# benfred/implicit

Measured on NVIDIA H100. Metric: ALS user+item row-updates/sec at f=64, higher is better.
Workload: dtype f32 (tensor-core accumulation with 3-term hi/lo splits, fp32-faithful)

## Files before the change

implicit_b200/csrc/cholesky_device.cuh:

```cuda
#pragma once
#include <limits.h>
#include <stdlib.h>

#include <cuda_fp16.h>

#include "common.h"

namespace als {

namespace {

__device__ __forceinline__ void mma_tf32(float (&d)[4], uint32_t a0, uint32_t a1, uint32_t a2, uint32_t a3,
                                         uint32_t b0, uint32_t b1) {
  asm volatile(
      "mma.sync.aligned.m16n8k8.row.col.f32.tf32.tf32.f32 {%0,%1,%2,%3}, {%4,%5,%6,%7}, {%8,%9}, {%0,%1,%2,%3};\n"
      : "+f"(d[0]), "+f"(d[1]), "+f"(d[2]), "+f"(d[3])
      : "r"(a0), "r"(a1), "r"(a2), "r"(a3), "r"(b0), "r"(b1));
}

__device__ __forceinline__ void cp_async16(float *smem_dst, const float *gmem_src) {
  const uint32_t s = (uint32_t)__cvta_generic_to_shared(smem_dst);
  asm volatile("cp.async.cg.shared.global [%0], [%1], 16;\n" ::"r"(s), "l"(gmem_src) : "memory");
}
__device__ __forceinline__ void cp_async_commit() { asm volatile("cp.async.commit_group;\n" ::: "memory"); }
template <int N>
__device__ __forceinline__ void cp_async_wait() {
  asm volatile("cp.async.wait_group %0;\n" ::"n"(N) : "memory");
}

constexpr uint32_t kTf32Mask = 0xffffe000u;
constexpr uint32_t kSignBit = 0x80000000u;

__device__ __forceinline__ uint32_t rn_tf32(float x) { return (__float_as_uint(x) + 0x1000u) & kTf32Mask; }
__device__ __forceinline__ void split_tf32(float x, uint32_t &hi, uint32_t &lo) {
  hi = rn_tf32(x);
  lo = __float_as_uint(x - __uint_as_float(hi));
}

__device__ __forceinline__ float rcp_approx(float x) {
  float r;
  asm("rcp.approx.ftz.f32 %0, %1;" : "=f"(r) : "f"(x));
  return r;
}
__device__ __forceinline__ float rsqrt_approx(float x) {
  float r;
  asm("rsqrt.approx.ftz.f32 %0, %1;" : "=f"(r) : "f"(x));
  return r;
}

template <int NB>
struct Cfg {
  static constexpr int F = 16 * NB;
  static constexpr int NT8 = 2 * NB;
  static constexpr int NTILES = NB * (NB + 1);
  static constexpr int LDS = F + 8;
  static constexpr int NSTAGE = 3;
  static constexpr int STAGE_FLOATS = 8 * LDS + 16;
  __host__ __device__ static constexpr int pstride(int p) { return F - 8 * p + ((p & 1) ? 0 : 8); }
  __host__ __device__ static constexpr int poff(int p) {
    int o = 0;
    for (int q = 0; q < p; ++q) o += 8 * pstride(q);
    return o;
  }
  static constexpr int U_FLOATS = poff(NT8);
  static constexpr int WARP_FLOATS = NSTAGE * STAGE_FLOATS + U_FLOATS + F ;
  __host__ __device__ static constexpr int tidx(int i, int j) { return i * NT8 - i * (i - 1) + (j - 2 * i); }
  static constexpr int SLOT_FLOATS = 32 * (NTILES * 4 + NT8);
};

constexpr int kWarpsPerCta = 1;

template <int NB>
struct RowState {
  float acc[Cfg<NB>::NTILES][4];
  float bp[Cfg<NB>::NT8];
};

struct Blk {
  int idx;
  float c;
};

__device__ __forceinline__ Blk load_block(const WorkItem &wi, int b, const int32_t *__restrict__ indices,
                                          const float *__restrict__ data, int lane) {
  const int k = wi.k0 + 32 * b + lane;
  const bool valid = k < wi.k1;
  Blk r;
  r.idx = valid ? __ldg(indices + k) : -1;
  r.c = valid ? __ldg(data + k) : 0.f;
  return r;
}

template <int NB>
__device__ __forceinline__ void issue_kstep(float *stage, const Blk &blk, int s, bool active,
                                            const float *__restrict__ Y, int lane) {
  using C = Cfg<NB>;
  if (active) {
    const int src = 8 * s + (lane & 7);
    const float c = __shfl_sync(0xffffffffu, blk.c, src);
    const int myidx = __shfl_sync(0xffffffffu, blk.idx, src);
    if (lane < 8) {
      const float w = (myidx >= 0) ? fabsf(c) - 1.f : 0.f;
      stage[8 * C::LDS + lane] = copysignf(__fsqrt_rn(fabsf(w)), w);
      stage[8 * C::LDS + 8 + lane] = (myidx >= 0 && c > 0.f) ? c : 0.f;
    }
    const int first = __shfl_sync(0xffffffffu, blk.idx, 8 * s);
    constexpr int CH = C::F / 4;
#pragma unroll
    for (int q = 0; q < NB; ++q) {
      const int id = q * 32 + lane;
      const int row = id / CH, ch = id % CH;
      int ridx = __shfl_sync(0xffffffffu, blk.idx, 8 * s + row);
      if (ridx < 0) ridx = first;
      cp_async16(stage + row * C::LDS + ch * 4, Y + (int64_t)ridx * C::F + ch * 4);
    }
  }
  cp_async_commit();
}

template <int NB>
__device__ __forceinline__ void consume_kstep(RowState<NB> &st, const float *stage, int g, int t) {
  using C = Cfg<NB>;
  const float s0 = stage[8 * C::LDS + t], s1 = stage[8 * C::LDS + t + 4];
  const float c0 = stage[8 * C::LDS + 8 + t], c1 = stage[8 * C::LDS + 8 + t + 4];
  const float a0 = fabsf(s0), a1 = fabsf(s1);
  const uint32_t m0 = __float_as_uint(s0) & kSignBit, m1 = __float_as_uint(s1) & kSignBit;
  uint32_t vh0[C::NT8], vl0[C::NT8], vh1[C::NT8], vl1[C::NT8];
#pragma unroll
  for (int c = 0; c < C::NT8; ++c) {
    const float y0 = stage[t * C::LDS + 8 * c + g];
    const float y1 = stage[(t + 4) * C::LDS + 8 * c + g];
    st.bp[c] = fmaf(c0, y0, st.bp[c]);
    st.bp[c] = fmaf(c1, y1, st.bp[c]);
    split_tf32(a0 * y0, vh0[c], vl0[c]);
    split_tf32(a1 * y1, vh1[c], vl1[c]);
  }
#pragma unroll
  for (int term = 0; term < 3; ++term) {
#pragma unroll
    for (int i = 0; i < NB; ++i) {
      const uint32_t a0 = (term == 0 ? vl0[2 * i] : vh0[2 * i]) ^ m0;
      const uint32_t a1 = (term == 0 ? vl0[2 * i + 1] : vh0[2 * i + 1]) ^ m0;
      const uint32_t a2 = (term == 0 ? vl1[2 * i] : vh1[2 * i]) ^ m1;
      const uint32_t a3 = (term == 0 ? vl1[2 * i + 1] : vh1[2 * i + 1]) ^ m1;
#pragma unroll
      for (int j = 2 * i; j < C::NT8; ++j) {
        float(&d)[4] = st.acc[C::tidx(i, j)];
        if (term == 1) mma_tf32(d, a0, a1, a2, a3, vl0[j], vl1[j]);
        else mma_tf32(d, a0, a1, a2, a3, vh0[j], vh1[j]);
      }
    }
  }
}

__device__ __forceinline__ void mma_f16(float (&d)[4], uint32_t a0, uint32_t a1, uint32_t a2, uint32_t a3, uint32_t b0,
                                        uint32_t b1) {
  asm volatile(
      "mma.sync.aligned.m16n8k16.row.col.f32.f16.f16.f32 {%0,%1,%2,%3}, {%4,%5,%6,%7}, {%8,%9}, {%0,%1,%2,%3};\n"
      : "+f"(d[0]), "+f"(d[1]), "+f"(d[2]), "+f"(d[3])
      : "r"(a0), "r"(a1), "r"(a2), "r"(a3), "r"(b0), "r"(b1));
}

__device__ __forceinline__ void split_f16_pair(float x0, float x1, uint32_t &hi, uint32_t &lo) {
  const __half2 h = __floats2half2_rn(x0, x1);
  const float2 hf = __half22float2(h);
  const __half2 l = __floats2half2_rn(x0 - hf.x, x1 - hf.y);
  hi = *reinterpret_cast<const uint32_t *>(&h);
  lo = *reinterpret_cast<const uint32_t *>(&l);
}

__device__ __forceinline__ float pow2_scale_below_2_14(float p) {
  const unsigned b = __float_as_uint(p);
  const int E = (int)(b >> 23) & 0xff;
  int se = (b & 0x7fffffffu) ? 267 - E : 127;
  se = se < 1 ? 1 : se > 253 ? 253 : se;
  return __uint_as_float((unsigned)se << 23);
}

template <int NB>
struct Cfg16 {
  using C = Cfg<NB>;
  static constexpr int F = C::F;
  static constexpr int LDS = F + 4;
  static constexpr int NSTAGE = 2;
  static constexpr int STAGE_FLOATS = 16 * LDS + 32;
  static constexpr int WARP_FLOATS = NSTAGE * STAGE_FLOATS + C::U_FLOATS + F ;
};

template <int NB>
__device__ __forceinline__ void issue_kstep16(float *stage, const Blk &blk, int s2, bool active, float sigma,
                                              const float *__restrict__ Y, int lane) {
  using C = Cfg16<NB>;
  if (active) {
    const int src = 16 * s2 + (lane & 15);
    const float c = __shfl_sync(0xffffffffu, blk.c, src);
    const int myidx = __shfl_sync(0xffffffffu, blk.idx, src);
    if (lane < 16) {
      const float w = (myidx >= 0) ? fabsf(c) - 1.f : 0.f;
      stage[16 * C::LDS + lane] = copysignf(sigma * __fsqrt_rn(fabsf(w)), w);
      stage[16 * C::LDS + 16 + lane] = (myidx >= 0 && c > 0.f) ? c : 0.f;
    }
    const int first = __shfl_sync(0xffffffffu, blk.idx, 16 * s2);
    constexpr int CH = C::F / 4;
#pragma unroll
    for (int q = 0; q < 2 * NB; ++q) {
      const int id = q * 32 + lane;
      const int row = id / CH, ch = id % CH;
      int ridx = __shfl_sync(0xffffffffu, blk.idx, 16 * s2 + row);
      if (ridx < 0) ridx = first;
      cp_async16(stage + row * C::LDS + ch * 4, Y + (int64_t)ridx * C::F + ch * 4);
    }
  }
  cp_async_commit();
}

template <int NB>
__device__ __forceinline__ void consume_kstep16(RowState<NB> &st, const float *stage, int g, int t) {
  using C = Cfg<NB>;
  constexpr int LDS = Cfg16<NB>::LDS;
  const float2 s0 = *reinterpret_cast<const float2 *>(stage + 16 * LDS + 2 * t);
  const float2 s1 = *reinterpret_cast<const float2 *>(stage + 16 * LDS + 2 * t + 8);
  const float2 c0 = *reinterpret_cast<const float2 *>(stage + 16 * LDS + 16 + 2 * t);
  const float2 c1 = *reinterpret_cast<const float2 *>(stage + 16 * LDS + 16 + 2 * t + 8);
  const float a00 = fabsf(s0.x), a01 = fabsf(s0.y), a10 = fabsf(s1.x), a11 = fabsf(s1.y);
  const uint32_t m0 = ((__float_as_uint(s0.x) >> 16) & 0x8000u) | (__float_as_uint(s0.y) & kSignBit);
  const uint32_t m1 = ((__float_as_uint(s1.x) >> 16) & 0x8000u) | (__float_as_uint(s1.y) & kSignBit);
  uint32_t h0[C::NT8], l0[C::NT8], h1[C::NT8], l1[C::NT8];
  const float *r00 = stage + (2 * t) * LDS + g, *r01 = r00 + LDS, *r10 = r00 + 8 * LDS, *r11 = r10 + LDS;
#pragma unroll
  for (int c = 0; c < C::NT8; ++c) {
    const float y00 = r00[8 * c], y01 = r01[8 * c], y10 = r10[8 * c], y11 = r11[8 * c];
    st.bp[c] = fmaf(c0.x, y00, st.bp[c]);
    st.bp[c] = fmaf(c0.y, y01, st.bp[c]);
    st.bp[c] = fmaf(c1.x, y10, st.bp[c]);
    st.bp[c] = fmaf(c1.y, y11, st.bp[c]);
    split_f16_pair(a00 * y00, a01 * y01, h0[c], l0[c]);
    split_f16_pair(a10 * y10, a11 * y11, h1[c], l1[c]);
  }
#pragma unroll
  for (int term = 0; term < 3; ++term) {
#pragma unroll
    for (int i = 0; i < NB; ++i) {
      const uint32_t a0 = (term == 0 ? l0[2 * i] : h0[2 * i]) ^ m0;
      const uint32_t a1 = (term == 0 ? l0[2 * i + 1] : h0[2 * i + 1]) ^ m0;
      const uint32_t a2 = (term == 0 ? l1[2 * i] : h1[2 * i]) ^ m1;
      const uint32_t a3 = (term == 0 ? l1[2 * i + 1] : h1[2 * i + 1]) ^ m1;
#pragma unroll
      for (int j = 2 * i; j < C::NT8; ++j) {
        float(&d)[4] = st.acc[C::tidx(i, j)];
        if (term == 1) mma_f16(d, a0, a1, a2, a3, l0[j], l1[j]);
        else mma_f16(d, a0, a1, a2, a3, h0[j], h1[j]);
      }
    }
  }
}

template <int NB>
__device__ __forceinline__ void factor_solve(RowState<NB> &st, float *U, float *zb, int lane, bool &ok, int dbg,
                                             float (&xx)[(Cfg<NB>::F + 31) / 32]) {
  using C = Cfg<NB>;
  constexpr int F = C::F;
  const int g = lane >> 2, t = lane & 3;

#pragma unroll
  for (int p = 0; p < C::NT8; ++p) {
    const int i = p >> 1, h = p & 1;
    float *Up = U + C::poff(p);
    const int sp = C::pstride(p);
    const int Wp = F - 8 * p;
    constexpr int NJmax = (F + 9 + 31) / 32;
    const int NJ = (Wp + 9 + 31) / 32;
#pragma unroll
    for (int j = p; j < C::NT8; ++j) {
      const float2 v = make_float2(st.acc[C::tidx(i, j)][2 * h], st.acc[C::tidx(i, j)][2 * h + 1]);
      *reinterpret_cast<float2 *>(Up + g * sp + 8 * (j - p) + 2 * t) = v;
    }
    {
      float bq = st.bp[p];
      bq += __shfl_xor_sync(0xffffffffu, bq, 1);
      bq += __shfl_xor_sync(0xffffffffu, bq, 2);
      if (t == 0) zb[8 * p + g] = bq;
    }
    __syncwarp();
    float v[NJmax][8];
#pragma unroll
    for (int j = 0; j < NJmax; ++j) {
      if (j < NJ) {
        const int c = lane + 32 * j;
        const float *colp = (c < Wp) ? (Up + c) : (zb + 8 * p);
        const int rs = (c < Wp) ? sp : 1;
        const int e = c - Wp - 1;
#pragma unroll
        for (int r = 0; r < 8; ++r) v[j][r] = (c <= Wp) ? colp[r * rs] : (e == r ? 1.f : 0.f);
      }
    }
    if (!(dbg & 2)) {
#pragma unroll
      for (int r = 0; r < 8; ++r) {
        const float d = v[0][r];
        float rc = rcp_approx(d);
        rc = rc * fmaf(-d, rc, 2.f);
        const float rinv = __shfl_sync(0xffffffffu, rc, r);
#pragma unroll
        for (int r2 = r + 1; r2 < 8; ++r2) {
          const float u = __shfl_sync(0xffffffffu, v[0][r], r2) * rinv;
#pragma unroll
          for (int j = 0; j < NJmax; ++j)
            if (j < NJ) v[j][r2] = fmaf(-u, v[j][r], v[j][r2]);
        }
      }
#pragma unroll
      for (int r = 0; r < 8; ++r) {
        const float d = __shfl_sync(0xffffffffu, v[0][r], r);
        float s = rsqrt_approx(d);
        s = s * fmaf(-0.5f * d * s, s, 1.5f);
#pragma unroll
        for (int j = 0; j < NJmax; ++j)
          if (j < NJ) v[j][r] *= s;
      }
    }
    __syncwarp();
#pragma unroll
    for (int j = 0; j < NJmax; ++j) {
      if (j < NJ) {
        const int c = lane + 32 * j;
        if (c >= 8 && c < Wp) {
#pragma unroll
          for (int r = 0; r < 8; ++r) Up[r * sp + c] = v[j][r];
        } else if (c == Wp) {
#pragma unroll
          for (int r = 0; r < 8; ++r) zb[8 * p + r] = v[j][r];
        } else if (c > Wp && c <= Wp + 8) {
          float *dst = Up + (c - Wp - 1) * sp;
          *reinterpret_cast<float4 *>(dst) = make_float4(v[j][0], v[j][1], v[j][2], v[j][3]);
          *reinterpret_cast<float4 *>(dst + 4) = make_float4(v[j][4], v[j][5], v[j][6], v[j][7]);
        }
      }
    }
    __syncwarp();
    if (p + 1 < C::NT8 && !(dbg & 4)) {
      const float z0 = zb[8 * p + t], z1 = zb[8 * p + t + 4];
      uint32_t uh0[C::NT8], ul0[C::NT8], uh1[C::NT8], ul1[C::NT8];
#pragma unroll
      for (int j = p + 1; j < C::NT8; ++j) {
        const float u0 = Up[t * sp + 8 * (j - p) + g];
        const float u1 = Up[(t + 4) * sp + 8 * (j - p) + g];
        st.bp[j] = fmaf(-u0, z0, st.bp[j]);
        st.bp[j] = fmaf(-u1, z1, st.bp[j]);
        split_tf32(u0, uh0[j], ul0[j]);
        split_tf32(u1, uh1[j], ul1[j]);
      }
#pragma unroll
      for (int term = 0; term < 3; ++term) {
#pragma unroll
        for (int ib = (p + 1) >> 1; ib < NB; ++ib) {
          const bool top = (2 * ib > p);
          const int jt = top ? 2 * ib : p + 1;
          const uint32_t a0 = top ? ((term == 0 ? ul0[jt] : uh0[jt]) ^ kSignBit) : 0u;
          const uint32_t a2 = top ? ((term == 0 ? ul1[jt] : uh1[jt]) ^ kSignBit) : 0u;
          const uint32_t a1 = (term == 0 ? ul0[2 * ib + 1] : uh0[2 * ib + 1]) ^ kSignBit;
          const uint32_t a3 = (term == 0 ? ul1[2 * ib + 1] : uh1[2 * ib + 1]) ^ kSignBit;
#pragma unroll
          for (int j = (2 * ib > p + 1 ? 2 * ib : p + 1); j < C::NT8; ++j) {
            float(&d)[4] = st.acc[C::tidx(ib, j)];
            if (term == 1) mma_tf32(d, a0, a1, a2, a3, ul0[j], ul1[j]);
            else mma_tf32(d, a0, a1, a2, a3, uh0[j], uh1[j]);
          }
        }
      }
    }
  }

  constexpr int Q = (F + 31) / 32;
  float zz[Q];
  int rowoff[Q];
#pragma unroll
  for (int q = 0; q < Q; ++q) {
    const int m = lane + 32 * q;
    const int mm = m < F ? m : 0;
    const int pm = mm >> 3;
    const int po = 8 * (pm * F - 4 * pm * (pm - 1) + 8 * ((pm + 1) >> 1));
    const int ps = F - 8 * pm + ((pm & 1) ? 0 : 8);
    rowoff[q] = po + (mm & 7) * ps - 8 * pm;
    zz[q] = zb[mm];
    xx[q] = 0.f;
  }
  if (!(dbg & 1))
#pragma unroll
  for (int p = C::NT8 - 1; p >= 0; --p) {
    const int qp = (8 * p) >> 5;
    const int l0 = (8 * p) & 31;
    const float4 da = *reinterpret_cast<const float4 *>(U + rowoff[qp] + 8 * p);
    const float4 db = *reinterpret_cast<const float4 *>(U + rowoff[qp] + 8 * p + 4);
    float rhs[8];
#pragma unroll
    for (int c = 0; c < 8; ++c) rhs[c] = __shfl_sync(0xffffffffu, zz[qp], l0 + c);
    const float xm = fmaf(da.x, rhs[0], fmaf(da.y, rhs[1], fmaf(da.z, rhs[2], da.w * rhs[3]))) +
                     fmaf(db.x, rhs[4], fmaf(db.y, rhs[5], fmaf(db.z, rhs[6], db.w * rhs[7])));
    const bool in_panel = (lane >= l0) && (lane < l0 + 8);
    if (in_panel) xx[qp] = xm;
    float xs[8];
#pragma unroll
    for (int c = 0; c < 8; ++c) xs[c] = __shfl_sync(0xffffffffu, xm, l0 + c);
#pragma unroll
    for (int q = 0; q < Q; ++q) {
      if (32 * q < 8 * p) {
        const int m = lane + 32 * q;
        if (m < 8 * p) {
          const float4 ua = *reinterpret_cast<const float4 *>(U + rowoff[q] + 8 * p);
          const float4 ub = *reinterpret_cast<const float4 *>(U + rowoff[q] + 8 * p + 4);
          const float s0 = fmaf(ua.x, xs[0], fmaf(ua.y, xs[1], fmaf(ua.z, xs[2], ua.w * xs[3])));
          const float s1 = fmaf(ub.x, xs[4], fmaf(ub.y, xs[5], fmaf(ub.z, xs[6], ub.w * xs[7])));
          zz[q] -= s0 + s1;
        }
      }
    }
  }
  bool fin = true;
#pragma unroll
  for (int q = 0; q < Q; ++q) {
    const int m = lane + 32 * q;
    if (m < F) {
      fin = fin && (fabsf(xx[q]) <= 3.0e38f);
    }
  }
  ok = __all_sync(0xffffffffu, fin);
}

template <int F>
__device__ __forceinline__ void store_solution(const float (&xx)[(F + 31) / 32], float *__restrict__ xout, int lane,
                                               float *const *peers, int n_peers, int64_t xoff) {
#pragma unroll
  for (int q = 0; q < (F + 31) / 32; ++q) {
    const int m = lane + 32 * q;
    if (m < F) {
      xout[m] = xx[q];
      for (int pi = 0; pi < n_peers; ++pi) peers[pi][xoff + m] = xx[q];
    }
  }
}

}

}
```

Baseline: 104.8 million.

## Factor 8x8 diagonal block per-lane and apply panel solve via TF32 mma

Replaces the warp-wide column-parallel elimination of each 8-row panel, which used many shuffles per pivot, with a redundant per-lane Cholesky of the 8x8 diagonal block. That step produces the inverse factor and the solved right-hand-side segment. The off-diagonal panel is then multiplied by this inverse using 3-term split TF32 mma tiles, and the results feed the trailing update directly from registers instead of being re-read from shared memory. This cuts shuffle latency and the serial dependency chain, at the cost of more register pressure (a 64-float matrix per lane) and a slightly different rounding path.

```diff
diff --git a/implicit_b200/csrc/cholesky_device.cuh b/implicit_b200/csrc/cholesky_device.cuh
--- a/implicit_b200/csrc/cholesky_device.cuh
+++ b/implicit_b200/csrc/cholesky_device.cuh
@@ -268,8 +268,6 @@
     float *Up = U + C::poff(p);
     const int sp = C::pstride(p);
     const int Wp = F - 8 * p;
-    constexpr int NJmax = (F + 9 + 31) / 32;
-    const int NJ = (Wp + 9 + 31) / 32;
 #pragma unroll
     for (int j = p; j < C::NT8; ++j) {
       const float2 v = make_float2(st.acc[C::tidx(i, j)][2 * h], st.acc[C::tidx(i, j)][2 * h + 1]);
@@ -282,69 +280,96 @@
       if (t == 0) zb[8 * p + g] = bq;
     }
     __syncwarp();
-    float v[NJmax][8];
-#pragma unroll
-    for (int j = 0; j < NJmax; ++j) {
-      if (j < NJ) {
-        const int c = lane + 32 * j;
-        const float *colp = (c < Wp) ? (Up + c) : (zb + 8 * p);
-        const int rs = (c < Wp) ? sp : 1;
-        const int e = c - Wp - 1;
-#pragma unroll
-        for (int r = 0; r < 8; ++r) v[j][r] = (c <= Wp) ? colp[r * rs] : (e == r ? 1.f : 0.f);
-      }
-    }
-    if (!(dbg & 2)) {
+    {
+      float a[8][8];
 #pragma unroll
       for (int r = 0; r < 8; ++r) {
-        const float d = v[0][r];
-        float rc = rcp_approx(d);
-        rc = rc * fmaf(-d, rc, 2.f);
-        const float rinv = __shfl_sync(0xffffffffu, rc, r);
-#pragma unroll
-        for (int r2 = r + 1; r2 < 8; ++r2) {
-          const float u = __shfl_sync(0xffffffffu, v[0][r], r2) * rinv;
-#pragma unroll
-          for (int j = 0; j < NJmax; ++j)
-            if (j < NJ) v[j][r2] = fmaf(-u, v[j][r], v[j][r2]);
-        }
-      }
-#pragma unroll
-      for (int r = 0; r < 8; ++r) {
-        const float d = __shfl_sync(0xffffffffu, v[0][r], r);
-        float s = rsqrt_approx(d);
-        s = s * fmaf(-0.5f * d * s, s, 1.5f);
-#pragma unroll
-        for (int j = 0; j < NJmax; ++j)
-          if (j < NJ) v[j][r] *= s;
-      }
-    }
-    __syncwarp();
-#pragma unroll
-    for (int j = 0; j < NJmax; ++j) {
-      if (j < NJ) {
-        const int c = lane + 32 * j;
-        if (c >= 8 && c < Wp) {
-#pragma unroll
-          for (int r = 0; r < 8; ++r) Up[r * sp + c] = v[j][r];
-        } else if (c == Wp) {
-#pragma unroll
-          for (int r = 0; r < 8; ++r) zb[8 * p + r] = v[j][r];
-        } else if (c > Wp && c <= Wp + 8) {
-          float *dst = Up + (c - Wp - 1) * sp;
-          *reinterpret_cast<float4 *>(dst) = make_float4(v[j][0], v[j][1], v[j][2], v[j][3]);
-          *reinterpret_cast<float4 *>(dst + 4) = make_float4(v[j][4], v[j][5], v[j][6], v[j][7]);
-        }
+        const float4 lo = *reinterpret_cast<const float4 *>(Up + r * sp);
+        const float4 hi = *reinterpret_cast<const float4 *>(Up + r * sp + 4);
+        a[r][0] = lo.x; a[r][1] = lo.y; a[r][2] = lo.z; a[r][3] = lo.w;
+        a[r][4] = hi.x; a[r][5] = hi.y; a[r][6] = hi.z; a[r][7] = hi.w;
+      }
+      float y[8];
+#pragma unroll
+      for (int r = 0; r < 8; ++r) y[r] = (lane == 8) ? zb[8 * p + r] : (lane == r ? 1.f : 0.f);
+      if (!(dbg & 2)) {
+#pragma unroll
+        for (int r = 0; r < 8; ++r) {
+          const float d = a[r][r];
+          float s = rsqrt_approx(d);
+          s = s * fmaf(-0.5f * d * s, s, 1.5f);
+#pragma unroll
+          for (int c = r + 1; c < 8; ++c) a[r][c] *= s;
+          y[r] *= s;
+#pragma unroll
+          for (int r2 = r + 1; r2 < 8; ++r2) {
+#pragma unroll
+            for (int c = r2; c < 8; ++c) a[r2][c] = fmaf(-a[r][r2], a[r][c], a[r2][c]);
+            y[r2] = fmaf(-a[r][r2], y[r], y[r2]);
+          }
+        }
+      }
+      __syncwarp();
+      if (lane < 8) {
+        float *dst = Up + lane * sp;
+        *reinterpret_cast<float4 *>(dst) = make_float4(y[0], y[1], y[2], y[3]);
+        *reinterpret_cast<float4 *>(dst + 4) = make_float4(y[4], y[5], y[6], y[7]);
+      } else if (lane == 8) {
+        *reinterpret_cast<float4 *>(zb + 8 * p) = make_float4(y[0], y[1], y[2], y[3]);
+        *reinterpret_cast<float4 *>(zb + 8 * p + 4) = make_float4(y[4], y[5], y[6], y[7]);
       }
     }
     __syncwarp();
     if (p + 1 < C::NT8 && !(dbg & 4)) {
-      const float z0 = zb[8 * p + t], z1 = zb[8 * p + t + 4];
+      constexpr int NMTmax = (F - 8 + 15) / 16;
+      const int NMT = (Wp - 8 + 15) / 16;
+      uint32_t bh[2], bl[2];
+      split_tf32(Up[t * sp + g], bh[0], bl[0]);
+      split_tf32(Up[(t + 4) * sp + g], bh[1], bl[1]);
+      uint32_t ah[NMTmax][4], al[NMTmax][4];
+      float d[NMTmax][4];
+#pragma unroll
+      for (int mt = 0; mt < NMTmax; ++mt) {
+        if (mt < NMT) {
+          const int m0 = 8 + 16 * mt + g, m1 = m0 + 8;
+          const bool in1 = m1 < Wp;
+          split_tf32(Up[t * sp + m0], ah[mt][0], al[mt][0]);
+          split_tf32(in1 ? Up[t * sp + m1] : 0.f, ah[mt][1], al[mt][1]);
+          split_tf32(Up[(t + 4) * sp + m0], ah[mt][2], al[mt][2]);
+          split_tf32(in1 ? Up[(t + 4) * sp + m1] : 0.f, ah[mt][3], al[mt][3]);
+          d[mt][0] = d[mt][1] = d[mt][2] = d[mt][3] = 0.f;
+        }
+      }
+#pragma unroll
+      for (int term = 0; term < 3; ++term) {
+#pragma unroll
+        for (int mt = 0; mt < NMTmax; ++mt) {
+          if (mt < NMT) {
+            const uint32_t(&a)[4] = term == 0 ? al[mt] : ah[mt];
+            const uint32_t(&b)[2] = term == 1 ? bl : bh;
+            mma_tf32(d[mt], a[0], a[1], a[2], a[3], b[0], b[1]);
+          }
+        }
+      }
+      __syncwarp();
+#pragma unroll
+      for (int mt = 0; mt < NMTmax; ++mt) {
+        if (mt < NMT) {
+          const int m0 = 8 + 16 * mt + g, m1 = m0 + 8;
+          Up[(2 * t) * sp + m0] = d[mt][0];
+          Up[(2 * t + 1) * sp + m0] = d[mt][1];
+          if (m1 < Wp) {
+            Up[(2 * t) * sp + m1] = d[mt][2];
+            Up[(2 * t + 1) * sp + m1] = d[mt][3];
+          }
+        }
+      }
+      const float z0 = zb[8 * p + 2 * t], z1 = zb[8 * p + 2 * t + 1];
       uint32_t uh0[C::NT8], ul0[C::NT8], uh1[C::NT8], ul1[C::NT8];
 #pragma unroll
       for (int j = p + 1; j < C::NT8; ++j) {
-        const float u0 = Up[t * sp + 8 * (j - p) + g];
-        const float u1 = Up[(t + 4) * sp + 8 * (j - p) + g];
+        const int jj = j - p - 1;
+        const float u0 = d[jj >> 1][2 * (jj & 1)], u1 = d[jj >> 1][2 * (jj & 1) + 1];
         st.bp[j] = fmaf(-u0, z0, st.bp[j]);
         st.bp[j] = fmaf(-u1, z1, st.bp[j]);
         split_tf32(u0, uh0[j], ul0[j]);
@@ -362,9 +387,9 @@
           const uint32_t a3 = (term == 0 ? ul1[2 * ib + 1] : uh1[2 * ib + 1]) ^ kSignBit;
 #pragma unroll
           for (int j = (2 * ib > p + 1 ? 2 * ib : p + 1); j < C::NT8; ++j) {
-            float(&d)[4] = st.acc[C::tidx(ib, j)];
-            if (term == 1) mma_tf32(d, a0, a1, a2, a3, ul0[j], ul1[j]);
-            else mma_tf32(d, a0, a1, a2, a3, uh0[j], uh1[j]);
+            float(&acc)[4] = st.acc[C::tidx(ib, j)];
+            if (term == 1) mma_tf32(acc, a0, a1, a2, a3, ul0[j], ul1[j]);
+            else mma_tf32(acc, a0, a1, a2, a3, uh0[j], uh1[j]);
           }
         }
       }
```

Result: faster. 106.2 million, median of 6 (+1.4%).
